# l-johnson-code/glTF-Renderer

Measured on AMD Instinct MI355X. Metric: Mrays/sec + ms/frame @1920x1080, 8-bounce, 1/2/4/8 MI355X, higher is better.
Workload: dtype f32

## Files before the change

### gltf_renderer_amd/csrc/pt_wavefront.hip

```cpp
#define PT_LUT_LDS 1
#include <type_traits>

#include "pt_vertex.h"
#include "pt_wavefront.h"
#include "pt_workspace.h"
#include "pt_bake.h"
#include "pt_probe.h"
#include "pt_matte.h"
#include "pt_motion.h"

#ifdef PT_TIMING
namespace pt { __device__ unsigned long long pt_timing[12]; }
extern "C" int pt_debug_read_timing(unsigned long long* out12, int reset) {
    hipDeviceSynchronize();
    hipMemcpyFromSymbol(out12, HIP_SYMBOL(pt::pt_timing), 96);
    if (reset) { unsigned long long z[12] = {0}; hipMemcpyToSymbol(HIP_SYMBOL(pt::pt_timing), z, 96); }
    return 0;
}
#endif
#ifdef PT_UTIL_PROBE
namespace pt { __device__ unsigned long long pt_util[16]; }
extern "C" int pt_debug_read_util(unsigned long long* out16, int reset) {
    hipDeviceSynchronize();
    hipMemcpyFromSymbol(out16, HIP_SYMBOL(pt::pt_util), 128);
    if (reset) { unsigned long long z[16] = {0}; hipMemcpyToSymbol(HIP_SYMBOL(pt::pt_util), z, 128); }
    return 0;
}
#define PT_UTIL(i, v) u_acc[i] += (v)
#else
#define PT_UTIL(i, v)
#endif
namespace pt {

typedef float nt_v4f __attribute__((ext_vector_type(4)));
PT_DEV float4 nt_load(const float4& p) { const nt_v4f v = __builtin_nontemporal_load((const nt_v4f*)&p); return make_float4(v.x, v.y, v.z, v.w); }
PT_DEV uint32_t nt_load(const uint32_t& p) { return __builtin_nontemporal_load(&p); }
PT_DEV void nt_store(float4& p, const float4 v) { nt_v4f q; q.x = v.x; q.y = v.y; q.z = v.z; q.w = v.w; __builtin_nontemporal_store(q, (nt_v4f*)&p); }
PT_DEV void nt_store(uint32_t& p, const uint32_t v) { __builtin_nontemporal_store(v, &p); }
#define QLD(p) nt_load(p)
#define QST(p, v) nt_store((p), (v))

#define PEND_ENV(s) wf.pend[2u * (s)]
#define PEND_LIGHT(s) wf.pend[2u * (s) + 1u]
constexpr int kRcAfterCamera = 1;

PT_DEV uint32_t queue_push(uint32_t* counter, bool pred) {
    const unsigned long long m = __ballot(pred);
    if (m == 0) return 0;
    const uint32_t lane = threadIdx.x & 63;
    const uint32_t rank = __popcll(m & ((1ull << lane) - 1ull));
    uint32_t base = 0;
    const int leader = __ffsll((long long)m) - 1;
    if ((int)lane == leader) base = atomicAdd(counter, (uint32_t)__popcll(m));
    base = __shfl(base, leader, 64);
    return base + rank;
}

struct ShardView { uint32_t shard, member, stride; };
PT_DEV ShardView shard_view(const WfBuffers& wf) {
    ShardView v;
    v.shard = blockIdx.x % kShards;
    v.member = blockIdx.x / kShards;
    v.stride = wf.blocks_per_shard * kBlock;
    return v;
}
static_assert((kTallyPrimary + kTallies) * 8 <= (int)kCounterStride * 4, "the tallies must fit the shard counter's line behind its word 0");
PT_DEV unsigned long long* shard_tallies(const WfBuffers& wf, uint32_t shard) { return (unsigned long long*)(wf.cnt[3] + shard * kCounterStride); }
PT_DEV void fold_shard_tallies(const WfBuffers& wf, Counters* __restrict__ counters) {
    if (blockIdx.x != 0 || threadIdx.x >= 64u) return;
    unsigned long long v[kTallies] = {0, 0, 0, 0, 0};
    for (uint32_t s = threadIdx.x; s < kShards; s += 64u) {
        const unsigned long long* t = shard_tallies(wf, s);
#pragma unroll
        for (int k = 0; k < kTallies; k++) v[k] += t[kTallyPrimary + k];
    }
    unsigned long long* c[kTallies] = {&counters->rays_primary, &counters->rays_bounce, &counters->rays_shadow, &counters->hits, &counters->taps};
#pragma unroll
    for (int k = 0; k < kTallies; k++) {
#pragma unroll
        for (int off = 32; off > 0; off >>= 1) v[k] += __shfl_down(v[k], off, 64);
        if (threadIdx.x == 0 && v[k]) atomicAdd(c[k], v[k]);
    }
}

PT_DEV bool adaptive_tile_active(const FrameConstants& fc, const AdaptiveArgs& ad, uint32_t slot0) {
    const uint32_t pair = slot0 >> 8;
    if (pair >= fc.my_tiles * fc.spp) return false;
    const uint32_t local_tile = pair - slot_sample(fc, slot0) * fc.my_tiles;
    return ad.tiles[local_tile].active != 0;
}
template <bool ADAPTIVE, bool LENS>
__global__ __launch_bounds__(kBlock) void k_wf_generate(FrameConstants fc, WfBuffers wf, Counters* __restrict__ counters, AdaptiveArgs ad, LensArgs lens) {
    if (!LENS) lens.enable = 0;
    const ShardView sv = shard_view(wf);
    const uint32_t per_xcd = gridDim.x / kXcds;
    const uint32_t xcd = blockIdx.x % kXcds, member = blockIdx.x / kXcds;
    uint32_t first_tile = xcd * wf.gen_region_tiles;
    uint32_t n_tiles = first_tile < fc.my_tiles ? min(wf.gen_region_tiles, fc.my_tiles - first_tile) : 0u;
    unsigned n_primary = 0;
    for (uint32_t rnd = 0; rnd < wf.gen_rounds; rnd++) {
        const uint32_t slot = (rnd * gridDim.x + blockIdx.x) * kBlock + threadIdx.x;
        const uint32_t sample = slot_sample(fc, slot);
        uint32_t px = 0, py = 0;
        bool valid = slot < wf.capacity && slot_pixel(fc, slot, px, py);
        if (ADAPTIVE) { const bool tile_on = adaptive_tile_active(fc, ad, (rnd * gridDim.x + blockIdx.x) * kBlock); valid = valid && tile_on; }
        int rc = 0;
        Ray ray;
        ray.o = v3(0); ray.d = v3(0, 0, 1); ray.tmin = 0; ray.tmax = 0;
        if (valid) ray = camera_ray(fc, lens, sample_seed(fc, sample), px, py, rc);
        const uint32_t idx = queue_push(wf.cnt[0] + sv.shard * kCounterStride, valid);
        if (valid) {
            const size_t e = (size_t)sv.shard * wf.seg_cap + idx;
            QST(wf.ray_o[0][e], make_float4(ray.o.x, ray.o.y, ray.o.z, ray.tmax));
            QST(wf.ray_d[0][e], make_float4(ray.d.x, ray.d.y, ray.d.z, __uint_as_float(slot)));
            n_primary++;
        }
    }
    flush_shard_tallies(shard_tallies(wf, sv.shard), threadIdx.x & 63, n_primary, 0, 0, 0, 0);
}

template <bool ADAPTIVE>
__global__ __launch_bounds__(kBlock) void k_wf_generate_bake(FrameConstants fc, WfBuffers wf, Counters* __restrict__ counters, AdaptiveArgs ad, BakeArgs bk, AovArgs av) {
    const ShardView sv = shard_view(wf);
    unsigned n_primary = 0;
    for (uint32_t rnd = 0; rnd < wf.gen_rounds; rnd++) {
        const uint32_t slot = (rnd * gridDim.x + blockIdx.x) * kBlock + threadIdx.x;
        const uint32_t sample = slot_sample(fc, slot);
        uint32_t px = 0, py = 0;
        bool valid = slot < wf.capacity && slot_pixel(fc, slot, px, py);
        if (ADAPTIVE) { const bool tile_on = adaptive_tile_active(fc, ad, (rnd * gridDim.x + blockIdx.x) * kBlock); valid = valid && tile_on; }
        int rc = 0;
        Ray ray;
        ray.o = v3(0); ray.d = v3(0, 0, 1); ray.tmin = 0; ray.tmax = 0;
        bool covered = false;
        if (valid) covered = bake_ray(fc, bk, sample_seed(fc, sample), px, py, rc, ray);
        const uint32_t idx = queue_push(wf.cnt[0] + sv.shard * kCounterStride, covered);
        if (covered) {
            const size_t e = (size_t)sv.shard * wf.seg_cap + idx;
            QST(wf.ray_o[0][e], make_float4(ray.o.x, ray.o.y, ray.o.z, ray.tmax));
            QST(wf.ray_d[0][e], make_float4(ray.d.x, ray.d.y, ray.d.z, __uint_as_float(slot)));
            n_primary++;
        } else if (valid) {
            const float4 zero = make_float4(0.0f, 0.0f, 0.0f, 0.0f);
            wf.L[slot] = zero;
            if (av.albedo) QST(av.rec_albedo[slot], zero);
            if (av.normal_depth) QST(av.rec_normal[slot], zero);
        }
    }
    flush_shard_tallies(shard_tallies(wf, sv.shard), threadIdx.x & 63, n_primary, 0, 0, 0, 0);
}

template <bool ADAPTIVE>
__global__ __launch_bounds__(kBlock, 7) void k_wf_generate_probe(FrameConstants fc, WfBuffers wf, Counters* __restrict__ counters, AdaptiveArgs ad, ProbeArgs pa, AovArgs av) {
    const ShardView sv = shard_view(wf);
    unsigned n_primary = 0;
    for (uint32_t rnd = 0; rnd < wf.gen_rounds; rnd++) {
        const uint32_t slot = (rnd * gridDim.x + blockIdx.x) * kBlock + threadIdx.x;
        const uint32_t sample = slot_sample(fc, slot);
        uint32_t px = 0, py = 0;
        bool valid = slot < wf.capacity && slot_pixel(fc, slot, px, py);
        if (ADAPTIVE) { const bool tile_on = adaptive_tile_active(fc, ad, (rnd * gridDim.x + blockIdx.x) * kBlock); valid = valid && tile_on; }
        int rc = 0;
        Ray ray;
        ray.o = v3(0); ray.d = v3(0, 0, 1); ray.tmin = 0; ray.tmax = 0;
        bool present = false;
        if (valid) present = probe_ray<true>(fc, pa, sample_seed(fc, sample), px, py, rc, ray);
        const uint32_t idx = queue_push(wf.cnt[0] + sv.shard * kCounterStride, present);
        if (present) {
            const size_t e = (size_t)sv.shard * wf.seg_cap + idx;
            QST(wf.ray_o[0][e], make_float4(ray.o.x, ray.o.y, ray.o.z, ray.tmax));
            QST(wf.ray_d[0][e], make_float4(ray.d.x, ray.d.y, ray.d.z, __uint_as_float(slot)));
            n_primary++;
        } else if (valid) {
            const float4 zero = make_float4(0.0f, 0.0f, 0.0f, 0.0f);
            wf.L[slot] = zero;
            if (av.albedo) QST(av.rec_albedo[slot], zero);
            if (av.normal_depth) QST(av.rec_normal[slot], zero);
        }
    }
    flush_shard_tallies(shard_tallies(wf, sv.shard), threadIdx.x & 63, n_primary, 0, 0, 0, 0);
}

#ifndef PT_REFILL
#define PT_REFILL 32
#endif
template <bool COUNT, int MODE>
PT_DEV void trace_persistent(const SceneRec& sc, const WfBuffers& wf, int* my_stack, const ShardView& sv, int cur, uint32_t rf_closest, uint32_t rmask,
                             uint32_t flags, LaneStats& st, float shadow_tmax = 0.0f) {
    const uint32_t n = wf.cnt[cur][sv.shard * kCounterStride];
    uint32_t* head = wf.cnt[MODE == 0 ? 3 : 4] + sv.shard * kCounterStride;
    const size_t base = MODE == 0 ? (size_t)sv.shard * wf.seg_cap : (size_t)sv.shard * wf.seg_cap * 2;
    const uint32_t lane = threadIdx.x & 63;
    int spill[kStackSpill];
    Trav t;
    t.cur = kTravDone; t.sp = 0;
    bool has = false, exhausted = (n == 0);
    uint32_t entry = 0, slot_bits = 0;
#ifdef PT_UTIL_PROBE
    unsigned long long u_acc[8] = {0, 0, 0, 0, 0, 0, 0, 0};
#endif
    for (;;) {
        const unsigned long long idle = __ballot(!has);
        const uint32_t nidle = (uint32_t)__popcll(idle);
        if (!exhausted && nidle >= PT_REFILL) {
            const int leader = __ffsll((long long)idle) - 1;
            uint32_t first = 0;
            if ((int)lane == leader) first = atomicAdd(head, nidle);
            first = __shfl(first, leader, 64);
            PT_UTIL(4, 1); PT_UTIL(5, min(nidle, first < n ? n - first : 0u));
            if (!has) {
                const uint32_t i = first + (uint32_t)__popcll(idle & ((1ull << lane) - 1ull));
                if (i < n) {
                    Ray ray;
                    if (MODE == 0) {
                        const float4 o = QLD(wf.ray_o[cur][base + i]), d = QLD(wf.ray_d[cur][base + i]);
                        ray.o = v3(o.x, o.y, o.z); ray.tmin = 0; ray.d = v3(d.x, d.y, d.z); ray.tmax = o.w;
                        trav_init(t, sc, ray, rf_closest, rmask, 0, 0.0f);
                    } else {
                        const float4 o = QLD(wf.sh_o[base + i]), d = QLD(wf.sh_d[base + i]);
                        slot_bits = __float_as_uint(o.w);
                        ray.o = v3(o.x, o.y, o.z); ray.tmin = 0; ray.d = v3(d.x, d.y, d.z); ray.tmax = shadow_tmax;
                        const bool alpha_shadow = (slot_bits >> 31) && (flags & PT_FLAG_ALPHA_SHADOWS);
                        uint32_t srf = (flags & PT_FLAG_CULL_BACKFACE) ? RF_CULL_BACK : 0;
                        srf |= alpha_shadow ? RF_FORCE_NON_OPAQUE : RF_ACCEPT_FIRST;
                        trav_init(t, sc, ray, srf, 0xff, 1, alpha_shadow ? 1.0f : 0.0f);
                    }
                    entry = i;
                    has = true;
                }
            }
            if (first + nidle >= n) exhausted = true;
        }
        if (__ballot(has) == 0) {
            if (exhausted) break;
            continue;
        }
#ifndef PT_NODE_MIN
#define PT_NODE_MIN 16
#endif
        for (;;) {
            const unsigned long long at_node = __ballot(has && t.cur >= 0);
            if (at_node == 0) break;
            if (PT_NODE_MIN > 1 && (int)__popcll(at_node) < PT_NODE_MIN && __ballot(has && t.cur < 0 && t.cur != kTravDone) != 0) break;
            PT_UTIL(0, 1); PT_UTIL(1, __popcll(at_node)); PT_UTIL(6, __popcll(__ballot(has)));
            if (has && t.cur >= 0) trav_node_step<COUNT, MODE == 0>(t, sc, my_stack, spill, st);
        }
#ifdef PT_UTIL_PROBE
        { const unsigned long long at_leaf = __ballot(has && t.cur != kTravDone && t.cur < 0); if (at_leaf) { PT_UTIL(2, 1); PT_UTIL(3, __popcll(at_leaf)); } }
#endif
        if (has && t.cur != kTravDone && t.cur < 0) trav_leaf_step<COUNT>(t, sc, my_stack, spill, st);
        if (has && t.cur == kTravDone) {
            if (MODE == 0) {
                const uint32_t bits = t.committed ? ((uint32_t)t.best.tri | (t.best.front ? 0x80000000u : 0u)) : kMissTri;
                QST(wf.hit[base + entry], make_float4(t.best.t, t.best.u, t.best.v, __uint_as_float(bits)));
            } else {
                const float tr = t.committed ? t.transmission : 1.0f;
                const uint32_t slot = slot_bits & 0x7fffffffu;
                float* w = (slot_bits >> 31) ? &PEND_LIGHT(slot).w : &PEND_ENV(slot).w;
                *w = tr;
            }
            has = false;
        }
    }
#ifdef PT_UTIL_PROBE
    if (lane == 0) for (int k = 0; k < 7; k++) atomicAdd(&pt_util[MODE * 8 + k], u_acc[k]);
#endif
}

PT_DEV bool env_prepass_wanted(const SceneRec& sc, const FrameConstants& fc, int vertex_bounce) {
    return sc.has_env && (fc.flags & PT_FLAG_ENVIRONMENT_MAP) && (fc.flags & PT_FLAG_ENVIRONMENT_MIS) && vertex_bounce < fc.max_bounces;
}
PT_DEV void env_prepass(const SceneRec& sc, const FrameConstants& fc, const WfBuffers& wf, int* stack_lds, const ShardView& sv, int cur, bool first_vertex) {
    static_assert((size_t)kStackLds * kBlock * sizeof(int) >= (size_t)kImpLdsFloat4 * sizeof(float4), "the traversal stack's LDS must hold the importance pyramid's coarse levels");
    float4* top = (float4*)stack_lds;
    stage_importance_top_into(sc, top);
    const uint32_t n = wf.cnt[cur][sv.shard * kCounterStride];
    const size_t base = (size_t)sv.shard * wf.seg_cap;
    for (uint32_t i = sv.member * kBlock + threadIdx.x; i < n; i += sv.stride) {
        const uint32_t slot = QLD(*((const uint32_t*)&wf.ray_d[cur][base + i] + 3));
        int rc = kRcAfterCamera;
        if (!first_vertex) rc = (int)(QLD(*((const uint32_t*)&wf.q_thr[cur][base + i] + 3)) & 0xffffu);
        uint32_t px, py;
        slot_pixel(fc, slot, px, py);
        const vec4 r = next_random(px, py, sample_seed(fc, slot_sample(fc, slot)), rc);
        const EnvSample e = environment_light_sample(sc, fc.environment_intensity, r.x, r.y, top);
        QST(wf.env_a[base + i], make_float4(e.dir.x, e.dir.y, e.dir.z, e.pdf));
        QST(wf.env_b[base + i], make_float4(e.color.x, e.color.y, e.color.z, 0.0f));
    }
    __syncthreads();
}

#ifndef PT_TRACE_WAVES
#define PT_TRACE_WAVES 1
#endif
constexpr uint32_t kTravFlagMask = PT_FLAG_CULL_BACKFACE | PT_FLAG_ALPHA_SHADOWS | PT_FLAG_INDIRECT_ENVIRONMENT_ONLY;
template <bool COUNT, bool DEFAULTS>
__global__ __launch_bounds__(kBlock, PT_TRACE_WAVES) void k_wf_trace(SceneRec sc, FrameConstants fc, WfBuffers wf, int cur, int bounce, uint32_t rf, uint32_t rmask, Counters* __restrict__ counters) {
    if (DEFAULTS) { rf = 0; rmask = 0xff; }
    __shared__ int s_stack[kStackLds * kBlock];
    stage_luts(sc);
    const ShardView sv = shard_view(wf);
    if (env_prepass_wanted(sc, fc, bounce)) env_prepass(sc, fc, wf, s_stack, sv, cur, bounce == 0);
    if (sv.member == 0 && threadIdx.x == 0) { wf.cnt[cur ^ 1][sv.shard * kCounterStride] = 0; wf.cnt[shadow_counter(bounce)][sv.shard * kCounterStride] = 0; wf.cnt[6][sv.shard * kCounterStride] = 0; }
    LaneStats st = {0, 0, 0, 0};
    trace_persistent<COUNT, 0>(sc, wf, s_stack + threadIdx.x, sv, cur, rf, rmask, 0, st);
    if (COUNT) { flush_counters(counters, threadIdx.x & 63, 0, 0, 0, 0, st); if (st.deep) atomicAdd(&counters->deep_pushes, (unsigned long long)st.deep); }
    else if (st.overflow | st.deep) flush_rare(counters, st);
}

template <bool COUNT, bool DEFAULTS>
__global__ __launch_bounds__(kBlock, PT_TRACE_WAVES) void k_wf_traverse(SceneRec sc, FrameConstants fc, WfBuffers wf, int nxt, int bounce, uint32_t rf, uint32_t rmask, uint32_t flags,
                                                                        Counters* __restrict__ counters) {
    if (DEFAULTS) { rf = 0; rmask = 0xff; flags &= ~kTravFlagMask; }
    __shared__ int s_stack[kStackLds * kBlock];
    stage_luts(sc);
    const ShardView sv = shard_view(wf);
    if (env_prepass_wanted(sc, fc, bounce + 1)) env_prepass(sc, fc, wf, s_stack, sv, nxt, false);
    if (sv.member == 0 && threadIdx.x == 0) { wf.cnt[nxt ^ 1][sv.shard * kCounterStride] = 0; wf.cnt[shadow_counter(bounce + 1)][sv.shard * kCounterStride] = 0; wf.cnt[6][sv.shard * kCounterStride] = 0; }
    LaneStats st_shadow = {0, 0, 0, 0}, st = {0, 0, 0, 0};
    trace_persistent<COUNT, 1>(sc, wf, s_stack + threadIdx.x, sv, shadow_counter(bounce), 0, 0xff, flags, st_shadow, fc.max_ray_length);
    trace_persistent<COUNT, 0>(sc, wf, s_stack + threadIdx.x, sv, nxt, rf, rmask, 0, st);
    if (COUNT) {
        flush_counters(counters, threadIdx.x & 63, 0, 0, 0, 0, st_shadow, true); flush_counters(counters, threadIdx.x & 63, 0, 0, 0, 0, st);
        if (st.deep | st_shadow.deep) atomicAdd(&counters->deep_pushes, (unsigned long long)st.deep + st_shadow.deep);
    } else if (st.overflow | st_shadow.overflow | st.deep | st_shadow.deep) { flush_rare(counters, st); flush_rare(counters, st_shadow); }
}

PT_DEV void apply_pending(const WfBuffers& wf, uint32_t slot, uint32_t pf, vec3& L) {
    const float4 pe = PEND_ENV(slot), pl = PEND_LIGHT(slot);
    if ((pf & 1u) && pe.w > 0.0f) L += v3(pe.x, pe.y, pe.z) * pe.w;
    if ((pf & 2u) && pl.w > 0.0f) L += v3(pl.x, pl.y, pl.z) * pl.w;
}

constexpr uint32_t kNoHeld = 0xffffffffu;
constexpr int kDeferFlush = 60;
constexpr uint32_t kDeferMajority = 4;
#ifndef PT_SHADE_WAVES
#define PT_SHADE_WAVES 2
#endif
constexpr uint32_t kShadeFlagMask = PT_FLAG_MATERIAL_DIFFUSE_WHITE | PT_FLAG_MATERIAL_MIS | PT_FLAG_MATERIAL_USE_GEOMETRIC_NORMALS | PT_FLAG_SHADING_NORMAL_ADAPTATION |
                                    PT_FLAG_ENVIRONMENT_MAP | PT_FLAG_ENVIRONMENT_MIS | PT_FLAG_INDIRECT_ENVIRONMENT_ONLY | PT_FLAG_POINT_LIGHTS | PT_FLAG_SHADOW_RAYS;
constexpr uint32_t kShadeSpecialised = 0x80000000u;
constexpr uint32_t kShadeDefaultsNoLights = PT_FLAG_SHADOW_RAYS | PT_FLAG_ENVIRONMENT_MAP | PT_FLAG_ENVIRONMENT_MIS | PT_FLAG_MATERIAL_MIS | PT_FLAG_SHADING_NORMAL_ADAPTATION;
constexpr uint32_t kShadeDefaults = kShadeDefaultsNoLights | PT_FLAG_POINT_LIGHTS;
template <uint32_t SPECIAL, bool SMALL>
__global__ __launch_bounds__(kBlock, PT_SHADE_WAVES) void k_wf_shade(SceneRec sc_in, FrameConstants fc_in, WfBuffers wf, int cur, int bounce, Counters* __restrict__ counters) {
    SceneRec sc = sc_in; sc.small_tables = SMALL ? 1u : 0u;
    FrameConstants fc = fc_in;
    if (SPECIAL) { fc.flags = (fc_in.flags & ~kShadeFlagMask) | (SPECIAL & kShadeFlagMask); fc.debug_output = PT_DEBUG_OUTPUT_NONE; }
    {
        const ShardView sv0 = shard_view(wf);
        if (sv0.member != 0 && sv0.member * kBlock >= wf.cnt[cur][sv0.shard * kCounterStride]) return;
    }
    stage_luts(sc);
    stage_tangent_lut(sc);
    stage_lights(sc, fc.num_of_lights);
    stage_instances(sc);
    stage_materials(sc);
    const ShardView sv = shard_view(wf);
    const uint32_t n = wf.cnt[cur][sv.shard * kCounterStride];
    const int nxt = cur ^ 1;
    const size_t base = (size_t)sv.shard * wf.seg_cap, sbase = (size_t)sv.shard * wf.seg_cap * 2;
    uint32_t* cnt_next = wf.cnt[nxt] + sv.shard * kCounterStride;
    uint32_t* cnt_shadow = wf.cnt[shadow_counter(bounce)] + sv.shard * kCounterStride;
    if (sv.member == 0 && threadIdx.x == 0) { wf.cnt[3][sv.shard * kCounterStride] = 0; wf.cnt[4][sv.shard * kCounterStride] = 0; }
    unsigned n_bounce = 0, n_shadow = 0, n_hits = 0;
    LaneStats st = {0, 0, 0, 0};
    uint32_t* shade_head = wf.cnt[6] + sv.shard * kCounterStride;
    const uint32_t lane64 = threadIdx.x & 63u;
    uint32_t chunk = 0;
    if (lane64 == 0) chunk = atomicAdd(shade_head, 64u);
    chunk = (uint32_t)__builtin_amdgcn_readfirstlane((int)chunk);
    const bool defer_on = false;
    uint32_t held = kNoHeld;
    __shared__ uint32_t s_hand[kBlock];
    uint32_t* hand = s_hand + (threadIdx.x & ~63u);
    __shared__ float2 s_park[2 * kBlock];
    const ParkLds park = {s_park + threadIdx.x};
    for (;;) {
        const bool more = chunk < n;
        const unsigned long long held_mask = __ballot(held != kNoHeld);
        if (!more && held_mask == 0) break;
        const bool flush = defer_on && (!more || __popcll(held_mask) >= kDeferFlush);
        uint32_t next_chunk = 0;
        if (!flush && lane64 == 0) next_chunk = atomicAdd(shade_head, 64u);
        const uint32_t i = flush ? held : chunk + lane64;
        const bool active = flush ? held != kNoHeld : i < n;
        if (flush) held = kNoHeld;
        bool push_env = false, push_light = false, push_bounce = false;
        Followups fu;
        fu.q_env = fu.q_light = fu.q_bounce = false;
        uint32_t slot = 0;
        PathState ps;
        ps.beta = v3(0); ps.thr = v3(0); ps.prev_pdf = 0; ps.rc = 0; ps.bounce = 0; ps.prev_mis = false;
        float4 o = make_float4(0, 0, 0, 0), d = o, h = o, bp = o, tm = o, Lq = o, pe = o, pl = o;
        uint32_t hb = kMissTri;
        const ShadePacket* packet_at = sc.shade;
        RawPacket packet;
        EnvSample es;
        es.dir = v3(0, 0, 1); es.pdf = 1; es.color = v3(0);
        const bool with_state = bounce != 0;
        if (active) {
            o = QLD(wf.ray_o[cur][base + i]); d = QLD(wf.ray_d[cur][base + i]); h = QLD(wf.hit[base + i]);
            if (env_prepass_wanted(sc, fc, bounce)) {
                const float4 ea = QLD(wf.env_a[base + i]), eb = QLD(wf.env_b[base + i]);
                es.dir = v3(ea.x, ea.y, ea.z); es.pdf = ea.w; es.color = v3(eb.x, eb.y, eb.z);
            }
            slot = __float_as_uint(d.w);
            hb = __float_as_uint(h.w);
#ifdef PT_PROBE_NO_PACKET
            packet_at = sc.shade + (hb == kMissTri ? 0u : (hb & 63u));
#else
            packet_at = sc.shade + (hb == kMissTri ? 0u : (hb & 0x7fffffffu));
#endif
            packet = load_shade_packet_raw(packet_at);
            if (with_state) {
                bp = QLD(wf.q_beta[cur][base + i]); tm = QLD(wf.q_thr[cur][base + i]);
#ifndef PT_PROBE_NO_LP
                Lq = wf.L[slot]; pe = PEND_ENV(slot); pl = PEND_LIGHT(slot);
#endif
            }
        }
        bool set_aside = false;
        if (defer_on && !flush) {
            const bool rare = false;
            const unsigned long long R = __ballot(rare), F = ~held_mask;
            const uint32_t nR = (uint32_t)__popcll(R), nF = (uint32_t)__popcll(F);
            if (nR != 0 && nR < kDeferMajority) {
                const unsigned long long below = (1ull << lane64) - 1ull;
                const uint32_t rr = (uint32_t)__popcll(R & below), rf = (uint32_t)__popcll(F & below);
                if (rare && rr < nF) { hand[rr] = i; set_aside = true; }
                __builtin_amdgcn_fence(__ATOMIC_RELEASE, "wavefront");
                __builtin_amdgcn_wave_barrier();
                __builtin_amdgcn_fence(__ATOMIC_ACQUIRE, "wavefront");
                if (held == kNoHeld && rf < min(nR, nF)) held = hand[rf];
            }
        }
        if (active && !set_aside) {
            Ray ray;
            ray.o = v3(o.x, o.y, o.z); ray.tmin = 0; ray.d = v3(d.x, d.y, d.z); ray.tmax = o.w;
            vec3 L = v3(0);
            ps.beta = v3(1); ps.prev_pdf = 0; ps.thr = v3(1); ps.rc = kRcAfterCamera; ps.bounce = 0; ps.prev_mis = false;
            if (with_state) {
                const uint32_t misc = __float_as_uint(tm.w);
                ps.beta = v3(bp.x, bp.y, bp.z); ps.prev_pdf = bp.w; ps.thr = v3(tm.x, tm.y, tm.z);
                ps.rc = (int)(misc & 0xffffu); ps.bounce = (int)((misc >> 16) & 0x7fffu); ps.prev_mis = (misc >> 31) != 0;
#ifndef PT_PROBE_NO_LP
                L = v3(Lq.x, Lq.y, Lq.z);
                const uint32_t pfb = __float_as_uint(Lq.w);
                if ((pfb & 1u) && pe.w > 0.0f) L += v3(pe.x, pe.y, pe.z) * pe.w;
                if ((pfb & 2u) && pl.w > 0.0f) L += v3(pl.x, pl.y, pl.z) * pl.w;
#endif
            }
            uint32_t pf = 0;
            if (hb == kMissTri) L += shade_miss(sc, fc, ray.d, ps);
            else {
                HitRec hit;
                hit.t = h.x; hit.u = h.y; hit.v = h.z; hit.tri = (int)(hb & 0x7fffffffu); hit.front = (hb >> 31) != 0;
                uint32_t px, py;
                slot_pixel(fc, slot, px, py);
                n_hits++;
                const bool done = shade_closest_hit<true>(sc, fc, sample_seed(fc, slot_sample(fc, slot)), px, py, ray, hit, packet, packet_at, ps, fu, st.taps, &es, park);
                if (fu.overwrite) L = v3(0);
                L += fu.add;
                n_shadow += fu.counted_shadow;
                if (!done) {
                    push_env = fu.q_env; push_light = fu.q_light; push_bounce = fu.q_bounce;
#ifndef PT_PROBE_NO_LP
                    if (push_env) { pf |= 1u; PEND_ENV(slot) = make_float4(fu.pend_env.x, fu.pend_env.y, fu.pend_env.z, 0.0f); }
                    if (push_light) { pf |= 2u; PEND_LIGHT(slot) = make_float4(fu.pend_light.x, fu.pend_light.y, fu.pend_light.z, 0.0f); }
#endif
                }
            }
#ifndef PT_PROBE_NO_LP
            wf.L[slot] = make_float4(L.x, L.y, L.z, __uint_as_float(pf));
#endif
        }
        const unsigned long long m_env = __ballot(push_env), m_light = __ballot(push_light), m_bounce = __ballot(push_bounce);
        const uint32_t c_env = (uint32_t)__popcll(m_env), c_shadow = c_env + (uint32_t)__popcll(m_light), c_bounce = (uint32_t)__popcll(m_bounce);
#ifdef PT_PROBE_ONE_WAIT
        uint32_t r_env = 0, r_light = 0, r_bounce = 0;
        if (m_env && (int)lane64 == __ffsll((long long)m_env) - 1) r_env = atomicAdd(cnt_shadow, c_env);
        if (m_light && (int)lane64 == __ffsll((long long)m_light) - 1) r_light = atomicAdd(cnt_shadow, c_shadow - c_env);
        if (m_bounce && (int)lane64 == __ffsll((long long)m_bounce) - 1) r_bounce = atomicAdd(cnt_next, c_bounce);
        const unsigned long long below = (1ull << lane64) - 1ull;
        const uint32_t ie = (m_env ? __shfl(r_env, __ffsll((long long)m_env) - 1, 64) : 0u) + (uint32_t)__popcll(m_env & below);
        const uint32_t il = (m_light ? __shfl(r_light, __ffsll((long long)m_light) - 1, 64) : 0u) + (uint32_t)__popcll(m_light & below);
        const uint32_t ib = (m_bounce ? __shfl(r_bounce, __ffsll((long long)m_bounce) - 1, 64) : 0u) + (uint32_t)__popcll(m_bounce & below);
#else
        uint32_t reserved = 0;
        if ((c_shadow | c_bounce) != 0u && lane64 < 2u) {
            const uint32_t add = lane64 == 0u ? c_shadow : c_bounce;
            if (add != 0u) reserved = atomicAdd(lane64 == 0u ? cnt_shadow : cnt_next, add);
        }
        const uint32_t base_shadow = (uint32_t)__builtin_amdgcn_readlane((int)reserved, 0), base_bounce = (uint32_t)__builtin_amdgcn_readlane((int)reserved, 1);
        const unsigned long long below = (1ull << lane64) - 1ull;
        const uint32_t ie = base_shadow + (uint32_t)__popcll(m_env & below);
        const uint32_t il = base_shadow + c_env + (uint32_t)__popcll(m_light & below);
        const uint32_t ib = base_bounce + (uint32_t)__popcll(m_bounce & below);
#endif
        if (push_env) {
            QST(wf.sh_o[sbase + ie], make_float4(fu.origin_above.x, fu.origin_above.y, fu.origin_above.z, __uint_as_float(slot)));
            QST(wf.sh_d[sbase + ie], make_float4(fu.env_dir.x, fu.env_dir.y, fu.env_dir.z, __uint_as_float(kNoHint)));
            n_shadow++;
        }
        if (push_light) {
            QST(wf.sh_o[sbase + il], make_float4(fu.origin_above.x, fu.origin_above.y, fu.origin_above.z, __uint_as_float(slot | 0x80000000u)));
            QST(wf.sh_d[sbase + il], make_float4(fu.light_dir.x, fu.light_dir.y, fu.light_dir.z, __uint_as_float(kNoHint)));
            n_shadow++;
        }
        if (push_bounce) {
            QST(wf.ray_o[nxt][base + ib], make_float4(fu.b_o.x, fu.b_o.y, fu.b_o.z, fc.max_ray_length));
            QST(wf.ray_d[nxt][base + ib], make_float4(fu.b_d.x, fu.b_d.y, fu.b_d.z, __uint_as_float(slot)));
            const uint32_t misc = ((uint32_t)ps.rc & 0xffffu) | ((uint32_t)(ps.bounce + 1) << 16) | (fu.b_mis ? 0x80000000u : 0u);
            QST(wf.q_beta[nxt][base + ib], make_float4(fu.b_beta.x, fu.b_beta.y, fu.b_beta.z, fu.b_pdf));
            QST(wf.q_thr[nxt][base + ib], make_float4(fu.b_thr.x, fu.b_thr.y, fu.b_thr.z, __uint_as_float(misc)));
            n_bounce++;
        }
        if (!flush) chunk = (uint32_t)__builtin_amdgcn_readfirstlane((int)next_chunk);
    }
    flush_shard_tallies(shard_tallies(wf, sv.shard), threadIdx.x & 63, 0, n_bounce, n_shadow, n_hits, st.taps);
}

template <bool COUNT>
__global__ __launch_bounds__(kBlock, PT_TRACE_WAVES) void k_wf_shadow(SceneRec sc, WfBuffers wf, int bounce, uint32_t flags, float tmax, Counters* __restrict__ counters) {
    __shared__ int s_stack[kStackLds * kBlock];
    stage_luts(sc);
    const ShardView sv = shard_view(wf);
    LaneStats st = {0, 0, 0, 0};
    trace_persistent<COUNT, 1>(sc, wf, s_stack + threadIdx.x, sv, shadow_counter(bounce), 0, 0xff, flags, st, tmax);
    if (COUNT) { flush_counters(counters, threadIdx.x & 63, 0, 0, 0, 0, st, true); if (st.deep) atomicAdd(&counters->deep_pushes, (unsigned long long)st.deep); }
    else if (st.overflow | st.deep) flush_rare(counters, st);
}

PT_DEV bool aov_finite(const float4 v) { return isfinite(v.x) && isfinite(v.y) && isfinite(v.z) && isfinite(v.w); }
__global__ __launch_bounds__(kBlock) void k_wf_aov(SceneRec sc_in, FrameConstants fc, WfBuffers wf, AovArgs av) {
    SceneRec sc = sc_in; sc.small_tables = 0u;
    const ShardView sv = shard_view(wf);
    const uint32_t n = wf.cnt[0][sv.shard * kCounterStride];
    if (sv.member * kBlock >= n) return;
    stage_luts(sc);
    stage_tangent_lut(sc);
    stage_instances(sc);
    stage_materials(sc);
    const size_t base = (size_t)sv.shard * wf.seg_cap;
    for (uint32_t i = sv.member * kBlock + threadIdx.x; i < n; i += sv.stride) {
        const float4 o = QLD(wf.ray_o[0][base + i]), d = QLD(wf.ray_d[0][base + i]), h = QLD(wf.hit[base + i]);
        const uint32_t slot = __float_as_uint(d.w), hb = __float_as_uint(h.w);
        float4 ra = make_float4(0, 0, 0, 0), rn = ra;
        if (hb != kMissTri) {
            const ShadePacket* packet_at = sc.shade + (hb & 0x7fffffffu);
            RawPacket packet = load_shade_packet_raw(packet_at);
            const ShadeInst inst = load_shade_inst(sc, raw_packet_inst(packet));
            if (inst.streams & (SI_TEXCOORD1 | SI_COLOR)) load_shade_packet_extra(packet, packet_at);
            const PacketVerts pv = unpack_shade_packet(packet);
            const RMat* mat = sc.rmats + inst.material_id;
            const MatHeader mh = material_header(sc, inst.material_id);
            HitGeom va = get_vertex_attributes(sc, inst, pv, v3(1 - h.y - h.z, h.y, h.z));
            if (!(hb >> 31)) { va.ng = -va.ng; va.n = -va.n; va.t = -va.t; va.tw = -va.tw; }
            const vec3 view = -normalize(v3(d.x, d.y, d.z));
            unsigned taps = 0;
            const Surface sp = get_surface(sc, fc.flags, mat, mh, va, view, taps);
            ra = make_float4(sp.albedo.x, sp.albedo.y, sp.albedo.z, 1.0f);
            rn = make_float4(sp.n.x, sp.n.y, sp.n.z, h.x);
            if (!aov_finite(ra)) ra = make_float4(0, 0, 0, 0);
            if (!aov_finite(rn)) rn = make_float4(0, 0, 0, 0);
        }
        if (av.albedo) QST(av.rec_albedo[slot], ra);
        if (av.normal_depth) QST(av.rec_normal[slot], rn);
    }
}
PT_DEV float4 blend_aov(float4 h, int accumulated, float4 v) {
    const float blend = fdiv(1.0f, (float)accumulated + 1.0f);
    return make_float4(h.x + blend * (v.x - h.x), h.y + blend * (v.y - h.y), h.z + blend * (v.z - h.z), h.w + blend * (v.w - h.w));
}
PT_DEV void resolve_aov_target(const FrameConstants& fc, const WfBuffers& wf, const float4* __restrict__ rec, float4* __restrict__ target, uint32_t pslot, size_t at, int first) {
    float4 pixel = make_float4(0, 0, 0, 0);
    if (first > 0) pixel = target[at];
    for (uint32_t k = 0; k < fc.spp; k++) {
        const float4 v = QLD(rec[k * fc.pixel_slots + pslot]);
        const int n = first + (int)k;
        pixel = n > 0 ? blend_aov(pixel, n, v) : v;
    }
    target[at] = pixel;
}
PT_DEV void resolve_aov(const FrameConstants& fc, const WfBuffers& wf, const AovArgs& av, uint32_t pslot, size_t at, int first) {
    if (av.albedo) resolve_aov_target(fc, wf, av.rec_albedo, av.albedo, pslot, at, first);
    if (av.normal_depth) resolve_aov_target(fc, wf, av.rec_normal, av.normal_depth, pslot, at, first);
}

PT_DEV float adaptive_pixel_error(const float4 I, const float4 A) {
    const float d = (fabsf(I.x - A.x) + fabsf(I.y - A.y)) + fabsf(I.z - A.z);
    const float s = (I.x + I.y) + I.z;
    const float e = d / (1e-4f + sqrtf(fmaxf(s, 0.0f)));
    return e != e ? INFINITY : e;
}
template <bool AOV>
PT_DEV void resolve_adaptive(const FrameConstants& fc, const WfBuffers& wf, float4* __restrict__ output, const AdaptiveArgs& ad, const AovArgs& av) {
    const uint32_t tile = blockIdx.x;
    if (ad.tiles[tile].active == 0) return;
    const uint32_t pslot = tile * kBlock + threadIdx.x;
    uint32_t px = 0, py = 0;
    const bool in_image = pslot < fc.pixel_slots && slot_pixel(fc, pslot, px, py);
    float e = -INFINITY;
    if (in_image) {
        const size_t at = (size_t)py * fc.res_x + px;
        float4 pixel = make_float4(0, 0, 0, 0), half = pixel;
        if (fc.accumulated_frames != 0) { pixel = output[at]; half = ad.half[at]; }
        for (uint32_t k = 0; k < fc.spp; k++) {
            const uint32_t slot = k * fc.pixel_slots + pslot;
            float4 Lq = wf.L[slot];
            vec3 L = v3(Lq.x, Lq.y, Lq.z);
            apply_pending(wf, slot, __float_as_uint(Lq.w), L);
            L = sanitize_sample(fc, L);
            const int n = fc.accumulated_frames + (int)k;
            pixel = n != 0 ? blend_sample(pixel, n, L) : make_float4(L.x, L.y, L.z, 1.0f);
            if ((n & 1) == 0) half = n != 0 ? blend_sample(half, n >> 1, L) : make_float4(L.x, L.y, L.z, 1.0f);
        }
        output[at] = pixel;
        ad.half[at] = half;
        e = adaptive_pixel_error(pixel, half);
        if (AOV) resolve_aov(fc, wf, av, pslot, at, fc.accumulated_frames);
    }
#pragma unroll
    for (int off = 32; off > 0; off >>= 1) e = fmaxf(e, __shfl_xor(e, off, 64));
    __shared__ float s_err[kBlock / 64];
    if ((threadIdx.x & 63u) == 0) s_err[threadIdx.x >> 6] = e;
    __syncthreads();
    if (threadIdx.x == 0) {
        float E = s_err[0];
#pragma unroll
        for (uint32_t w = 1; w < kBlock / 64; w++) E = fmaxf(E, s_err[w]);
        const int n = fc.accumulated_frames + (int)fc.spp;
        const bool retire = n >= ad.cap || (n >= ad.min_samples && E <= ad.threshold);
        AdaptiveTile t;
        t.active = retire ? 0u : 1u; t.samples = (uint32_t)n; t.error = E; t.pad = 0;
        ad.tiles[tile] = t;
    }
}

template <bool ADAPTIVE, bool AOV>
__global__ __launch_bounds__(kBlock) void k_wf_resolve(FrameConstants fc, WfBuffers wf, float4* __restrict__ output, AdaptiveArgs ad, AovArgs av, Counters* __restrict__ counters) {
    fold_shard_tallies(wf, counters);
    if (ADAPTIVE) { resolve_adaptive<AOV>(fc, wf, output, ad, av); return; }
    const uint32_t pslot = blockIdx.x * kBlock + threadIdx.x;
    uint32_t px, py;
    if (pslot >= fc.pixel_slots || !slot_pixel(fc, pslot, px, py)) return;
    float4* outp = output + ((size_t)py * fc.res_x + px);
    const bool accumulate = (fc.flags & PT_FLAG_ACCUMULATE) != 0;
    float4 pixel = make_float4(0, 0, 0, 0);
    if (accumulate && fc.accumulated_frames != 0) pixel = *outp;
    for (uint32_t k = 0; k < fc.spp; k++) {
        const uint32_t slot = k * fc.pixel_slots + pslot;
        float4 Lq = wf.L[slot];
        vec3 L = v3(Lq.x, Lq.y, Lq.z);
        apply_pending(wf, slot, __float_as_uint(Lq.w), L);
        L = sanitize_sample(fc, L);
        const int accumulated = fc.accumulated_frames + (int)k;
        pixel = (accumulate && accumulated != 0) ? blend_sample(pixel, accumulated, L) : make_float4(L.x, L.y, L.z, 1.0f);
    }
    *outp = pixel;
    if (AOV) resolve_aov(fc, wf, av, pslot, (size_t)py * fc.res_x + px, accumulate ? fc.accumulated_frames : -1);
}

__global__ __launch_bounds__(kBlock) void k_wf_matte(SceneRec sc, WfBuffers wf, MatteArgs ma) {
    const ShardView sv = shard_view(wf);
    const uint32_t n = wf.cnt[0][sv.shard * kCounterStride];
    const size_t base = (size_t)sv.shard * wf.seg_cap;
    for (uint32_t i = sv.member * kBlock + threadIdx.x; i < n; i += sv.stride) {
        const uint32_t slot = QLD(((const uint32_t*)(wf.ray_d[0] + base + i))[3]), hb = QLD(((const uint32_t*)(wf.hit + base + i))[3]);
        uint32_t id = 0u;
        if (hb != kMissTri) {
            uint32_t row = sc.shade[hb & 0x7fffffffu].inst;
            if (ma.kind == PT_MATTE_MATERIAL) row = sc.instances[row].gpu.material_id;
            if (row < ma.n_ids) id = ma.ids[row];
        }
        if (slot < wf.capacity) QST(ma.rec[slot], id);
    }
}
template <int RANKS, bool ADAPTIVE>
__global__ __launch_bounds__(kBlock) void k_wf_matte_resolve(FrameConstants fc, AdaptiveArgs ad, MatteArgs ma) {
    if (ADAPTIVE) { if (ad.tiles[blockIdx.x].active == 0) return; }
    const uint32_t pslot = blockIdx.x * kBlock + threadIdx.x;
    uint32_t px, py;
    if (pslot >= fc.pixel_slots || !slot_pixel(fc, pslot, px, py)) return;
    const size_t at = (size_t)py * fc.res_x + px;
    const bool accumulate = ADAPTIVE || (fc.flags & PT_FLAG_ACCUMULATE) != 0;
    const int first = accumulate ? fc.accumulated_frames : -1;
    MatteRanks<RANKS> m;
#pragma unroll
    for (int j = 0; j < RANKS / 2; j++) matte_unpack(m, j, first > 0 ? ma.layers[j][at] : make_float4(0.0f, 0.0f, 0.0f, 0.0f));
    for (uint32_t k = 0; k < fc.spp; k++) {
        const uint32_t h = QLD(ma.rec[k * fc.pixel_slots + pslot]);
        matte_fold_sample(m, h, first < 0 ? 0 : first + (int)k);
    }
    matte_sort(m);
#pragma unroll
    for (int j = 0; j < RANKS / 2; j++) ma.layers[j][at] = matte_pack(m, j);
}

__global__ __launch_bounds__(kBlock) void k_wf_motion(SceneRec sc, WfBuffers wf, MotionArgs ma) {
    const ShardView sv = shard_view(wf);
    const uint32_t n = wf.cnt[0][sv.shard * kCounterStride];
    const size_t base = (size_t)sv.shard * wf.seg_cap;
    for (uint32_t i = sv.member * kBlock + threadIdx.x; i < n; i += sv.stride) {
        const uint32_t slot = QLD(((const uint32_t*)(wf.ray_d[0] + base + i))[3]);
        const float4 h = QLD(wf.hit[base + i]);
        const uint32_t hb = __float_as_uint(h.w), tri = hb & 0x7fffffffu;
        float4 r = make_float4(0.0f, 0.0f, 0.0f, 0.0f);
        if (hb != kMissTri && tri < sc.num_tris) r = motion_record(sc, ma, tri, h.y, h.z);
        if (slot < wf.capacity) QST(ma.rec[slot], r);
    }
}
template <bool ADAPTIVE>
__global__ __launch_bounds__(kBlock) void k_wf_motion_resolve(FrameConstants fc, WfBuffers wf, AdaptiveArgs ad, MotionArgs ma) {
    if (ADAPTIVE) { if (ad.tiles[blockIdx.x].active == 0) return; }
    const uint32_t pslot = blockIdx.x * kBlock + threadIdx.x;
    uint32_t px, py;
    if (pslot >= fc.pixel_slots || !slot_pixel(fc, pslot, px, py)) return;
    const bool accumulate = ADAPTIVE || (fc.flags & PT_FLAG_ACCUMULATE) != 0;
    resolve_aov_target(fc, wf, ma.rec, ma.target, pslot, (size_t)py * fc.res_x + px, accumulate ? fc.accumulated_frames : -1);
}

PT_DEV float variance_finite_or_zero(float q) { return isfinite(q) ? q : 0.0f; }
template <bool ADAPTIVE>
__global__ __launch_bounds__(kBlock) void k_wf_variance_resolve(FrameConstants fc, WfBuffers wf, const float4* __restrict__ output, AdaptiveArgs ad, VarianceArgs va) {
    if (ADAPTIVE) { if (ad.tiles[blockIdx.x].active == 0) return; }
    const uint32_t pslot = blockIdx.x * kBlock + threadIdx.x;
    uint32_t px, py;
    if (pslot >= fc.pixel_slots || !slot_pixel(fc, pslot, px, py)) return;
    const size_t at = (size_t)py * fc.res_x + px;
    const bool accumulate = ADAPTIVE || (fc.flags & PT_FLAG_ACCUMULATE) != 0;
    const int first = accumulate ? fc.accumulated_frames : 0;
    float4 m = make_float4(0, 0, 0, 0), V = m;
    if (first > 0) { m = output[at]; V = va.target[at]; }
    for (uint32_t k = 0; k < fc.spp; k++) {
        const uint32_t slot = k * fc.pixel_slots + pslot;
        const float4 Lq = wf.L[slot];
        vec3 x = v3(Lq.x, Lq.y, Lq.z);
        apply_pending(wf, slot, __float_as_uint(Lq.w), x);
        x = sanitize_sample(fc, x);
        const int n = first + (int)k;
        if (n == 0) { V = make_float4(0, 0, 0, 0); m = make_float4(x.x, x.y, x.z, 1.0f); continue; }
        const float b = fdiv(1.0f, (float)n + 1.0f);
        const float4 mn = blend_sample(m, n, x);
        const vec3 d0 = v3(x.x - m.x, x.y - m.y, x.z - m.z), d1 = v3(x.x - mn.x, x.y - mn.y, x.z - mn.z);
        const float qr = variance_finite_or_zero(d0.x * d1.x), qg = variance_finite_or_zero(d0.y * d1.y), qb = variance_finite_or_zero(d0.z * d1.z);
        const float s0 = (d0.x + d0.y) + d0.z, s1 = (d1.x + d1.y) + d1.z;
        const float qs = variance_finite_or_zero(s0 * s1);
        V = make_float4(V.x + b * (qr - V.x), V.y + b * (qg - V.y), V.z + b * (qb - V.z), V.w + b * (qs - V.w));
        m = mn;
    }
    va.target[at] = V;
}

size_t wavefront_workspace_bytes(const FrameConstants& fc, int stage_blocks, const WavefrontPasses& passes) {
    return workspace_layout(fc.my_tiles, fc.spp, stage_blocks, passes.records(), kBlock).total;
}

static WfBuffers carve(void* workspace, const WorkspaceLayout& l, uint32_t slots) {
    auto at = [&](size_t offset) { return (float4*)((char*)workspace + offset); };
    WfBuffers wf;
    wf.chunks_per_shard = l.chunks_per_shard; wf.blocks_per_shard = l.blocks_per_shard; wf.seg_cap = l.seg_cap;
    wf.gen_region_tiles = 0; wf.gen_rounds = l.gen_rounds;
    for (int k = 0; k < kCounterArrays; k++) wf.cnt[k] = (uint32_t*)at(l.cnt[k]);
    wf.L = at(l.L); wf.beta_pdf = at(l.beta_pdf); wf.thr_misc = at(l.thr_misc); wf.pend = at(l.pend);
    for (int k = 0; k < 2; k++) { wf.ray_o[k] = at(l.ray_o[k]); wf.ray_d[k] = at(l.ray_d[k]); wf.q_beta[k] = at(l.q_beta[k]); wf.q_thr[k] = at(l.q_thr[k]); }
    wf.hit = at(l.hit); wf.env_a = at(l.env_a); wf.env_b = at(l.env_b); wf.sh_o = at(l.sh_o); wf.sh_d = at(l.sh_d);
    wf.sh_c = nullptr; wf.occ_cache = nullptr; wf.capacity = slots;
    return wf;
}

int traversal_stack_capacity() { return kStackLds + kStackSpill; }
size_t traversal_grid_lanes(int stage_blocks) { return (size_t)kShards * blocks_per_shard_for(stage_blocks) * kBlock; }

static bool traversal_defaults(uint32_t flags) { return (flags & kTravFlagMask) == 0; }
template <class F> static void pick(bool a, F&& f) { if (a) f(std::true_type()); else f(std::false_type()); }
template <class F> static void pick2(bool a, bool b, F&& f) { pick(a, [&](auto A) { pick(b, [&](auto B) { f(A, B); }); }); }
void launch_wf_trace(dim3 grid, hipStream_t stream, bool count, const SceneRec& sc, const FrameConstants& fc, const WfBuffers& w, int cur, int b, uint32_t rf,
                     uint32_t rmask, Counters* counters) {
    pick2(count, traversal_defaults(fc.flags), [&](auto COUNT, auto DEFAULTS) { hipLaunchKernelGGL((k_wf_trace<COUNT.value, DEFAULTS.value>), grid, dim3(kBlock), 0, stream, sc, fc, w, cur, b, rf, rmask, counters); });
}
void launch_wf_traverse(dim3 grid, hipStream_t stream, bool count, const SceneRec& sc, const FrameConstants& fc, const WfBuffers& w, int nxt, int b, uint32_t rf,
                        uint32_t rmask, Counters* counters) {
    pick2(count, traversal_defaults(fc.flags), [&](auto COUNT, auto DEFAULTS) { hipLaunchKernelGGL((k_wf_traverse<COUNT.value, DEFAULTS.value>), grid, dim3(kBlock), 0, stream, sc, fc, w, nxt, b, rf, rmask, fc.flags, counters); });
}
void launch_wf_shadow(dim3 grid, hipStream_t stream, bool count, const SceneRec& sc, const WfBuffers& w, int b, uint32_t flags, float tmax, Counters* counters) {
    pick(count, [&](auto COUNT) { hipLaunchKernelGGL(k_wf_shadow<COUNT.value>, grid, dim3(kBlock), 0, stream, sc, w, b, flags, tmax, counters); });
}

hipError_t launch_wavefront(const SceneRec& sc, const FrameConstants& fc, const LensArgs& lens, float4* output, Counters* counters, bool count, void* workspace,
                            int stage_blocks, StageTimers* timers, hipStream_t stream, const WavefrontPasses& passes) {
    if (timers) timers->used = 0;
    if (fc.my_tiles == 0) return hipSuccess;
    auto event_at = [&](size_t i) -> hipEvent_t {
        while (timers->ev.size() <= i) { hipEvent_t e = nullptr; if (hipEventCreate(&e) != hipSuccess) return nullptr; timers->ev.push_back(e); }
        return timers->ev[i];
    };
    auto mark = [&](int kind) {
        if (!timers) return;
        const size_t k = timers->used;
        hipEvent_t ev = event_at(k + 1);
        if (!ev) return;
        if (timers->kind.size() < k + 1) timers->kind.resize(k + 1);
        timers->kind[k] = (uint8_t)kind;
        hipEventRecord(ev, stream);
        timers->used = k + 1;
    };
    const uint32_t slots = fc.my_tiles * kBlock * fc.spp;
    const WorkspaceLayout lay = workspace_layout(fc.my_tiles, fc.spp, stage_blocks, passes.records(), kBlock);
    WfBuffers wf = carve(workspace, lay, slots);
    hipError_t e = hipMemsetAsync(wf.cnt[0], 0, (size_t)kCounterArrays * kShards * kCounterStride * 4, stream);
    if (e) return e;
    const dim3 block(kBlock), full(fc.my_tiles), stage(kShards * wf.blocks_per_shard);
    if (timers) { hipEvent_t ev = event_at(0); if (ev) hipEventRecord(ev, stream); else timers = nullptr; }
    const bool adaptive = passes.adaptive, aov = passes.aov, matte = passes.matte, motion = passes.motion;
    const AdaptiveArgs ad = adaptive ? passes.ad : AdaptiveArgs{};
    AovArgs av = aov ? passes.av : AovArgs{};
    MatteArgs mt = matte ? passes.mt : MatteArgs{};
    MotionArgs mo = motion ? passes.mo : MotionArgs{};
    if (aov) { av.rec_albedo = (float4*)((char*)workspace + lay.rec_albedo); av.rec_normal = (float4*)((char*)workspace + lay.rec_normal); }
    if (matte) {
        mt.rec = (uint32_t*)((char*)workspace + lay.rec_matte);
        if ((e = hipMemsetAsync(mt.rec, 0, (size_t)slots * 4, stream)) != hipSuccess) return e;
// ... 85 lines not shown
```

Measured before the change: 7053.

## Prefetch next shade chunk's hit and slot into LDS asynchronously

The shade kernel now uses global_load_lds to prefetch the next chunk's hit record and ray slot word into LDS while the current chunk is shaded. The work-queue atomic for the chunk after next is folded into the existing per-wave atomic reservation for shadow and bounce counters. The goal is to hide the dependent hit-to-packet load latency at the top of each iteration and to drop one separate atomic round trip per chunk. In exchange it uses extra LDS, adds explicit waitcnt barriers that may serialize the output stores, and reserves chunks one step earlier, which could unbalance work at the tail.

```diff
diff --git a/gltf_renderer_amd/csrc/pt_wavefront.hip b/gltf_renderer_amd/csrc/pt_wavefront.hip
--- a/gltf_renderer_amd/csrc/pt_wavefront.hip
+++ b/gltf_renderer_amd/csrc/pt_wavefront.hip
@@ -17,6 +17,11 @@
     if (reset) { unsigned long long z[12] = {0}; hipMemcpyToSymbol(HIP_SYMBOL(pt::pt_timing), z, 96); }
     return 0;
 }
+#define PT_WAIT_BEGIN() unsigned long long _a = __builtin_readcyclecounter();
+#define PT_WAIT_STAMP(K) { asm volatile("s_waitcnt vmcnt(0)" ::: "memory"); const unsigned long long _b = __builtin_readcyclecounter(); _wait[K] += _b - _a; _a = _b; }
+#else
+#define PT_WAIT_BEGIN()
+#define PT_WAIT_STAMP(K)
 #endif
 #ifdef PT_UTIL_PROBE
 namespace pt { __device__ unsigned long long pt_util[16]; }
@@ -39,6 +44,12 @@
 PT_DEV void nt_store(uint32_t& p, const uint32_t v) { __builtin_nontemporal_store(v, &p); }
 #define QLD(p) nt_load(p)
 #define QST(p, v) nt_store((p), (v))
+#define PT_LDS_FETCH(src, wave_base, BYTES, POLICY) \
+    __builtin_amdgcn_global_load_lds((const __attribute__((address_space(1))) void*)(src), (__attribute__((address_space(3))) void*)(wave_base), BYTES, 0, POLICY)
+PT_DEV void lds_fetch_queue(const float4* src, float4* wave_base) { PT_LDS_FETCH(src, wave_base, 16, 2); }
+PT_DEV void lds_fetch_queue(const uint32_t* src, uint32_t* wave_base) { PT_LDS_FETCH(src, wave_base, 4, 2); }
+PT_DEV void wait_vector_memory() { __builtin_amdgcn_s_waitcnt(0x0f70); asm volatile("" ::: "memory"); }
+PT_DEV void wait_lds() { asm volatile("" ::: "memory"); __builtin_amdgcn_s_waitcnt(0xc07f); asm volatile("" ::: "memory"); }
 
 #define PEND_ENV(s) wf.pend[2u * (s)]
 #define PEND_LIGHT(s) wf.pend[2u * (s) + 1u]
@@ -343,6 +354,13 @@
 constexpr uint32_t kShadeSpecialised = 0x80000000u;
 constexpr uint32_t kShadeDefaultsNoLights = PT_FLAG_SHADOW_RAYS | PT_FLAG_ENVIRONMENT_MAP | PT_FLAG_ENVIRONMENT_MIS | PT_FLAG_MATERIAL_MIS | PT_FLAG_SHADING_NORMAL_ADAPTATION;
 constexpr uint32_t kShadeDefaults = kShadeDefaultsNoLights | PT_FLAG_POINT_LIGHTS;
+PT_DEV const ShadePacket* packet_of(const SceneRec& sc, uint32_t hb) {
+#ifdef PT_PROBE_NO_PACKET
+    return sc.shade + (hb == kMissTri ? 0u : (hb & 63u));
+#else
+    return sc.shade + (hb == kMissTri ? 0u : (hb & 0x7fffffffu));
+#endif
+}
 template <uint32_t SPECIAL, bool SMALL>
 __global__ __launch_bounds__(kBlock, PT_SHADE_WAVES) void k_wf_shade(SceneRec sc_in, FrameConstants fc_in, WfBuffers wf, int cur, int bounce, Counters* __restrict__ counters) {
     SceneRec sc = sc_in; sc.small_tables = SMALL ? 1u : 0u;
@@ -368,22 +386,40 @@
     LaneStats st = {0, 0, 0, 0};
     uint32_t* shade_head = wf.cnt[6] + sv.shard * kCounterStride;
     const uint32_t lane64 = threadIdx.x & 63u;
-    uint32_t chunk = 0;
+    __shared__ float4 s_pre[kBlock + kBlock / 4];
+    const uint32_t wave_lane0 = (uint32_t)__builtin_amdgcn_readfirstlane((int)(threadIdx.x & ~63u));
+    float4* const pre_wave = s_pre + wave_lane0;
+    uint32_t* const pre_slot_wave = (uint32_t*)(s_pre + kBlock) + wave_lane0;
+    const auto lane_bytes = [&]() { uint32_t l = lane64; asm volatile("" : "+v"(l)); return l * 16u; };
+    const auto fetch_entry = [&](uint32_t c, uint32_t lb) {
+        if (c + lane64 < n) {
+            lds_fetch_queue((const float4*)((const char*)(wf.hit + base + c) + lb), pre_wave);
+            lds_fetch_queue((const uint32_t*)((const char*)(wf.ray_d[cur] + base + c) + 12 + lb), pre_slot_wave);
+        }
+    };
+    uint32_t chunk = 0, next_chunk = 0;
     if (lane64 == 0) chunk = atomicAdd(shade_head, 64u);
     chunk = (uint32_t)__builtin_amdgcn_readfirstlane((int)chunk);
+    if (chunk < n) {
+        if (lane64 == 0) next_chunk = atomicAdd(shade_head, 64u);
+        fetch_entry(chunk, lane_bytes());
+        wait_vector_memory();
+    }
+    next_chunk = (uint32_t)__builtin_amdgcn_readfirstlane((int)next_chunk);
     const bool defer_on = false;
     uint32_t held = kNoHeld;
     __shared__ uint32_t s_hand[kBlock];
     uint32_t* hand = s_hand + (threadIdx.x & ~63u);
     __shared__ float2 s_park[2 * kBlock];
     const ParkLds park = {s_park + threadIdx.x};
+#ifdef PT_TIMING
+    unsigned long long _wait[3] = {0, 0, 0};
+#endif
     for (;;) {
         const bool more = chunk < n;
         const unsigned long long held_mask = __ballot(held != kNoHeld);
         if (!more && held_mask == 0) break;
         const bool flush = defer_on && (!more || __popcll(held_mask) >= kDeferFlush);
-        uint32_t next_chunk = 0;
-        if (!flush && lane64 == 0) next_chunk = atomicAdd(shade_head, 64u);
         const uint32_t i = flush ? held : chunk + lane64;
         const bool active = flush ? held != kNoHeld : i < n;
         if (flush) held = kNoHeld;
@@ -400,19 +436,21 @@
         EnvSample es;
         es.dir = v3(0, 0, 1); es.pdf = 1; es.color = v3(0);
         const bool with_state = bounce != 0;
+        const uint32_t lb = lane_bytes();
         if (active) {
-            o = QLD(wf.ray_o[cur][base + i]); d = QLD(wf.ray_d[cur][base + i]); h = QLD(wf.hit[base + i]);
+            h = *(const float4*)((const char*)pre_wave + lb); slot = *(const uint32_t*)((const char*)pre_slot_wave + lb / 4u);
+        }
+        wait_lds();
+        fetch_entry(next_chunk, lb);
+        if (active) {
+            PT_WAIT_BEGIN()
+            o = QLD(wf.ray_o[cur][base + i]); d = QLD(wf.ray_d[cur][base + i]);
             if (env_prepass_wanted(sc, fc, bounce)) {
                 const float4 ea = QLD(wf.env_a[base + i]), eb = QLD(wf.env_b[base + i]);
                 es.dir = v3(ea.x, ea.y, ea.z); es.pdf = ea.w; es.color = v3(eb.x, eb.y, eb.z);
             }
-            slot = __float_as_uint(d.w);
             hb = __float_as_uint(h.w);
-#ifdef PT_PROBE_NO_PACKET
-            packet_at = sc.shade + (hb == kMissTri ? 0u : (hb & 63u));
-#else
-            packet_at = sc.shade + (hb == kMissTri ? 0u : (hb & 0x7fffffffu));
-#endif
+            packet_at = packet_of(sc, hb);
             packet = load_shade_packet_raw(packet_at);
             if (with_state) {
                 bp = QLD(wf.q_beta[cur][base + i]); tm = QLD(wf.q_thr[cur][base + i]);
@@ -420,6 +458,10 @@
                 Lq = wf.L[slot]; pe = PEND_ENV(slot); pl = PEND_LIGHT(slot);
 #endif
             }
+            PT_WAIT_STAMP(0)
+#ifdef PT_TIMING
+            _wait[2]++;
+#endif
         }
         bool set_aside = false;
         if (defer_on && !flush) {
@@ -476,6 +518,7 @@
             wf.L[slot] = make_float4(L.x, L.y, L.z, __uint_as_float(pf));
 #endif
         }
+        const bool reserve_chunk = !flush && next_chunk < n;
         const unsigned long long m_env = __ballot(push_env), m_light = __ballot(push_light), m_bounce = __ballot(push_bounce);
         const uint32_t c_env = (uint32_t)__popcll(m_env), c_shadow = c_env + (uint32_t)__popcll(m_light), c_bounce = (uint32_t)__popcll(m_bounce);
 #ifdef PT_PROBE_ONE_WAIT
@@ -487,18 +530,23 @@
         const uint32_t ie = (m_env ? __shfl(r_env, __ffsll((long long)m_env) - 1, 64) : 0u) + (uint32_t)__popcll(m_env & below);
         const uint32_t il = (m_light ? __shfl(r_light, __ffsll((long long)m_light) - 1, 64) : 0u) + (uint32_t)__popcll(m_light & below);
         const uint32_t ib = (m_bounce ? __shfl(r_bounce, __ffsll((long long)m_bounce) - 1, 64) : 0u) + (uint32_t)__popcll(m_bounce & below);
+        uint32_t r_head = 0;
+        if (reserve_chunk && lane64 == 0) r_head = atomicAdd(shade_head, 64u);
+        const uint32_t chunk_after_next = reserve_chunk ? (uint32_t)__builtin_amdgcn_readfirstlane((int)r_head) : next_chunk;
 #else
         uint32_t reserved = 0;
-        if ((c_shadow | c_bounce) != 0u && lane64 < 2u) {
-            const uint32_t add = lane64 == 0u ? c_shadow : c_bounce;
-            if (add != 0u) reserved = atomicAdd(lane64 == 0u ? cnt_shadow : cnt_next, add);
+        if (lane64 < 3u) {
+            const uint32_t add = lane64 == 0u ? c_shadow : (lane64 == 1u ? c_bounce : (reserve_chunk ? 64u : 0u));
+            if (add != 0u) reserved = atomicAdd(lane64 == 0u ? cnt_shadow : (lane64 == 1u ? cnt_next : shade_head), add);
         }
         const uint32_t base_shadow = (uint32_t)__builtin_amdgcn_readlane((int)reserved, 0), base_bounce = (uint32_t)__builtin_amdgcn_readlane((int)reserved, 1);
+        const uint32_t chunk_after_next = reserve_chunk ? (uint32_t)__builtin_amdgcn_readlane((int)reserved, 2) : next_chunk;
         const unsigned long long below = (1ull << lane64) - 1ull;
         const uint32_t ie = base_shadow + (uint32_t)__popcll(m_env & below);
         const uint32_t il = base_shadow + c_env + (uint32_t)__popcll(m_light & below);
         const uint32_t ib = base_bounce + (uint32_t)__popcll(m_bounce & below);
 #endif
+        wait_vector_memory();
         if (push_env) {
             QST(wf.sh_o[sbase + ie], make_float4(fu.origin_above.x, fu.origin_above.y, fu.origin_above.z, __uint_as_float(slot)));
             QST(wf.sh_d[sbase + ie], make_float4(fu.env_dir.x, fu.env_dir.y, fu.env_dir.z, __uint_as_float(kNoHint)));
@@ -517,9 +565,12 @@
             QST(wf.q_thr[nxt][base + ib], make_float4(fu.b_thr.x, fu.b_thr.y, fu.b_thr.z, __uint_as_float(misc)));
             n_bounce++;
         }
-        if (!flush) chunk = (uint32_t)__builtin_amdgcn_readfirstlane((int)next_chunk);
+        if (!flush) { chunk = next_chunk; next_chunk = chunk_after_next; }
     }
     flush_shard_tallies(shard_tallies(wf, sv.shard), threadIdx.x & 63, 0, n_bounce, n_shadow, n_hits, st.taps);
+#ifdef PT_TIMING
+    if (lane64 == 0) { for (int k = 0; k < 3; k++) atomicAdd(&pt_timing[8 + k], _wait[k]); }
+#endif
 }
 
 template <bool COUNT>
```

Result: faster. 7144, median of 6 (+1.3%).
